# PaddleCV-SIG/MedicalSeg

Measured on AMD Instinct MI355X. Metric: 3D-voxels/sec fwd+bwd, VNet 128^3 fp32, higher is better.
Workload: dtype f32

## Files before the change

### medicalseg_amd/csrc/msk_common.h

```cpp
#pragma once
#include <hip/hip_runtime.h>
#include <hip/hip_ext.h>

#include <cstdint>
#include <cstdio>
#include <cstring>
#include <map>
#include <set>
#include <string>
#include <utility>
#include <vector>

#include "msegk.h"

struct msk_prof_entry {
  double total_ms = 0.0;
  long calls = 0;
};

struct msk_pending_event {
  hipEvent_t a, b;
  const char* tag;
};

// ... 28 lines not shown
  std::set<const void*> xform_ok;
  bool conv_fp16 = false;
  int wbf_tin_map = 1;
  int wbf_mr4 = 1;
  int wbf_variant = -1;
  int halo_tile = -1;
  int wgrad_chunk = -1;
  char prof_prefix[48] = {0};
  long wgrad_async_max_m = 0;
  float* scalar_ring = nullptr;
  int scalar_next = 0;
  long scalar_served = 0;
  float* scalar_ring_side = nullptr;
  int scalar_next_side = 0;
  long scalar_served_side = 0;
  int wbf_tpb = 0;
  void* wpack = nullptr;
  int wbf_pack_cache = 1;
  void* spack = nullptr;
  int wbf_pack_lds = 1;
  int wbf_bpf = 1;
  int wbf_ks_blocks = 2;
  int noop_after_merge = 0;
  int wgrad_c1_wpc = 2;
  int eager_tail_main = 1;
  int prof_paused = 0;
  int prof_attach = 1;
  int small_pack_cache = 1;
  int wbf_prepack = 1;
  int ks_legacy = 0;
  int wgrad_fork = 1;
  int wbf_fused_bl = 2;
  int wbf_fuse = 1;
  int conv_split = 2;
  int bwd_fuse = -1;
  int foldn_wgs = 0;
  int wgrad_wino_rounds = 0;
  int wgrad_rounds = 8;
  int poison = -1;
  hipStream_t side = nullptr;
  void* ws_side = nullptr;
  size_t ws_side_bytes = 0;
  void* ws3_side = nullptr;
  size_t ws3_side_bytes = 0;
  hipEvent_t ev_fork = nullptr, ev_join = nullptr;
  hipEvent_t ev_late = nullptr;
  bool late_valid = false;
  const float* late_ptr = nullptr;
  size_t late_count = 0;
  float* late_alpha = nullptr;
  struct { float* param = nullptr; const float* grad = nullptr; float* velocity = nullptr; size_t count = 0;
           float lr = 0, momentum = 0, weight_decay = 0, grad_scale = 0; } late_piece;
  int late_split = 1;
  bool wgrad_async = false;
  bool side_dirty = false;
  hipEvent_t fork_event = nullptr;
  int fork_attach = 1;
  bool fork_recorded = false;
  void* stage[2] = {nullptr, nullptr};
  size_t stage_bytes[2] = {0, 0};
  hipEvent_t stage_ev[2] = {nullptr, nullptr};
  int stage_next = 0;
  void* comm = nullptr;
  void* comm_grad = nullptr;
  hipStream_t comm_stream = nullptr;
  hipEvent_t ev_comm_main = nullptr, ev_comm_side = nullptr, ev_comm_done = nullptr, ev_comm_back = nullptr;
  int c1_h2 = 1;
  int dst_split = 1;
  int wgrad_reduce_rows = 1;
  int ks_stats = 1;
  int ks_lds = 1;
  int ks_nr_max = 4;
  int wgrad_lds_pad = 0;
  int kst_pair = 1;
  int tile_staging = 7;
  int wgrad_renorm = 1;
  int dy_bound_shift = 0;
  int dp_mode = 0;
  bool comm_pending = false;
  bool host_transport = false;
  std::vector<int> host_fds;
  int rank = 0, world = 1;
  int tk_join = 1;
  int affine_map = 1;
  int num_cu = 256;
};

extern thread_local std::string g_msk_global_err;

int msk_fail(msk_ctx* ctx, const char* file, int line, const char* what, const char* detail);
void* msk_workspace(msk_ctx* ctx, size_t bytes);
void* msk_workspace2(msk_ctx* ctx, size_t bytes);
void* msk_workspace3(msk_ctx* ctx, size_t bytes);
hipEvent_t msk_prof_event(msk_ctx* ctx);
void msk_prof_begin(msk_ctx* ctx, const char* tag);
void msk_prof_end(msk_ctx* ctx);
const char* msk_intern_tag(msk_ctx* ctx, const std::string& s);
int msk_join_side_impl(msk_ctx* ctx);
void msk_set_dense12(int v);
void msk_set_reduce_vpl(int v);
void msk_set_reduce_vpl_site(int v);
void msk_set_ew_caps(int ew, int red);
void msk_weights_changed_impl(msk_ctx* ctx, const void* p, size_t bytes);
void msk_weights_freed_impl(msk_ctx* ctx, const void* p, size_t bytes);
int msk_wbf_prepack_impl(msk_ctx* ctx);
int msk_wbf_prepack_range_impl(msk_ctx* ctx, const void* p, size_t bytes);
void msk_wbf_pack_cache_free(msk_ctx* ctx);
void msk_small_pack_changed(msk_ctx* ctx, const void* p, size_t bytes);
void msk_small_pack_freed(msk_ctx* ctx, const void* p, size_t bytes);
int msk_small_prepack(msk_ctx* ctx, const void* p, size_t bytes);
void msk_small_pack_free(msk_ctx* ctx);
int msk_dp_wait_impl(msk_ctx* ctx);
int msk_join_sums_merge(msk_ctx* ctx, const float* partial, int nb, int C, float* unit_sums, float* u_dbeta, float* u_dgamma,
                        float* u_dalpha, float* dalpha);

struct msk_side_scope {
  msk_ctx* ctx;
  bool active;
  explicit msk_side_scope(msk_ctx* c, bool want = true) : ctx(c), active(want && c->wgrad_async && c->side != nullptr) {
    const bool forked = ctx->fork_recorded;
    hipEvent_t fev = forked && ctx->fork_event ? ctx->fork_event : ctx->ev_fork;
    ctx->fork_recorded = false;
    ctx->fork_event = nullptr;
    if (!active) return;
    if (!forked) hipEventRecord(ctx->ev_fork, ctx->stream);
    hipStreamWaitEvent(ctx->side, fev, 0);
    std::swap(ctx->stream, ctx->side);
    std::swap(ctx->ws, ctx->ws_side);
    std::swap(ctx->ws_bytes, ctx->ws_side_bytes);
    std::swap(ctx->ws3, ctx->ws3_side);
    std::swap(ctx->ws3_bytes, ctx->ws3_side_bytes);
    std::swap(ctx->scalar_ring, ctx->scalar_ring_side);
    std::swap(ctx->scalar_next, ctx->scalar_next_side);
    std::swap(ctx->scalar_served, ctx->scalar_served_side);
    ctx->side_dirty = true;
  }
  ~msk_side_scope() {
    if (!active) return;
    std::swap(ctx->stream, ctx->side);
    std::swap(ctx->ws, ctx->ws_side);
    std::swap(ctx->ws_bytes, ctx->ws_side_bytes);
    std::swap(ctx->ws3, ctx->ws3_side);
    std::swap(ctx->ws3_bytes, ctx->ws3_side_bytes);
    std::swap(ctx->scalar_ring, ctx->scalar_ring_side);
    std::swap(ctx->scalar_next, ctx->scalar_next_side);
    std::swap(ctx->scalar_served, ctx->scalar_served_side);
  }
};

#define MSK_CHECK_HIP(ctx, expr)                                                        \
  do {                                                                                  \
    hipError_t _e = (expr);                                                             \
    if (_e != hipSuccess) return msk_fail(ctx, __FILE__, __LINE__, #expr, hipGetErrorString(_e)); \
  } while (0)

#define MSK_REQUIRE(ctx, cond, msg)                                       \
  do {                                                                    \
    if (!(cond)) return msk_fail(ctx, __FILE__, __LINE__, #cond, msg);    \
  } while (0)

static inline bool msk_prof_selected(const msk_ctx* c, const char* tag) {
  return c->prof && ((!c->prof_paused && (c->prof_prefix[0] == 0 || strncmp(tag, c->prof_prefix, strlen(c->prof_prefix)) == 0)) ||
                     strncmp(tag, "rccl_", 5) == 0);
}
struct msk_launch_scope {
  msk_ctx* ctx;
// ... 78 lines not shown
```

### medicalseg_amd/csrc/msk_conv_foldn.hip

```cpp
#include "msk_conv.h"
#include "msk_wbf.h"

typedef _Float16 fn_f16x8 __attribute__((ext_vector_type(8)));

namespace {

struct FNArgs {
  const float* src;
  int sld;
  float* dst;
  int dld;
  int N, D, H, W, CN;
  const float4* wb;
  const float* bias;
  const float* prelu;
  int accumulate;
  int tiles_h, tiles_w, segs, seg_len, nblk;
  unsigned src_bytes;
};

__device__ __forceinline__ int xcd_remap_fn(int bid, int nb) {
  const int q = nb >> 3, r = nb & 7;
  const int xcd = bid & 7, idx = bid >> 3;
  return (xcd < r ? xcd * (q + 1) : r * (q + 1) + (xcd - r) * q) + idx;
// ... 262 lines not shown
  };

  const int tap0 = wave == 0 ? 0 : NT0 - NT1 + NT1 * wave, ntap = wave == 0 ? NT0 : NT1;
  uint4 bh[NT0], bl[NT0];
  int aoff[NT0];
#pragma unroll
  for (int j = 0; j < NT0; ++j) {
    const int tp = min(tap0 + j, 24);
    bh[j] = a.wb[(tp * 2 + 0) * 64 + lane];
    bl[j] = a.wb[(tp * 2 + 1) * 64 + lane];
    aoff[j] = (tp / 5) * HW + (tp % 5);
  }
  const int abase = lk * NV + li;

  const int col_co = li / 5, col_kd = li - col_co * 5;
  const bool col_live = li < 5 * a.CN;
  const bool col_first = col_kd == 0 || !col_live;
  f32x4 acc[TH];
#pragma unroll
  for (int r = 0; r < TH; ++r) acc[r] = (f32x4){0.f, 0.f, 0.f, 0.f};

  const int steps = (d_end - d_begin) + 4;
  fetch(d_begin - 2);
#pragma unroll 1
  for (int s = 0; s < steps; ++s) {
    const int dp = d_begin - 2 + s;
    const bool live = dp >= 0 && dp < a.D;
    __syncthreads();
    if (live) {
      char* lb = reinterpret_cast<char*>(lds);
#pragma unroll
      for (int j = 0; j < NLD; ++j)
        if (st_lds[j] >= 0) {
          uint2 hv, lv;
          wbf_split2h_pair(pre[j].x * sx, pre[j].y * sx, hv.x, lv.x);
          wbf_split2h_pair(pre[j].z * sx, pre[j].w * sx, hv.y, lv.y);
          *reinterpret_cast<uint2*>(lb + st_lds[j]) = hv;
          *reinterpret_cast<uint2*>(lb + PP * 16 + st_lds[j]) = lv;
        }
    }
    __syncthreads();
    if (s + 1 < steps) fetch(dp + 1);

#pragma unroll
    for (int r = 0; r < TH; ++r)
#pragma unroll
      for (int e = 0; e < 4; ++e) {
        const float cur = acc[r][e];
        const int sh = __builtin_amdgcn_update_dpp(0, __float_as_int(cur), 0x111 , 0xF, 0xF, true);
        acc[r][e] = col_first ? 0.f : __int_as_float(sh);
      }
    if (live) {
#pragma unroll
      for (int j = 0; j < NT0; ++j) {
        if (j < ntap) {
          const uint4* ap = lds + abase + aoff[j];
#pragma unroll
          for (int r = 0; r < TH; ++r) {
            const uint4 ah = ap[r * HW], al = ap[PP + r * HW];
            acc[r] = __builtin_amdgcn_mfma_f32_16x16x32_f16(__builtin_bit_cast(fn_f16x8, al), __builtin_bit_cast(fn_f16x8, bh[j]), acc[r], 0, 0, 0);
            acc[r] = __builtin_amdgcn_mfma_f32_16x16x32_f16(__builtin_bit_cast(fn_f16x8, ah), __builtin_bit_cast(fn_f16x8, bl[j]), acc[r], 0, 0, 0);
            acc[r] = __builtin_amdgcn_mfma_f32_16x16x32_f16(__builtin_bit_cast(fn_f16x8, ah), __builtin_bit_cast(fn_f16x8, bh[j]), acc[r], 0, 0, 0);
          }
        }
      }
    }
    const int d = dp - 2;
    const bool out_plane = d >= d_begin && d < d_end;
    if (out_plane && col_live && col_kd == 4) {
#pragma unroll
      for (int r = 0; r < TH; ++r)
#pragma unroll
        for (int e = 0; e < 4; ++e) red[wave][(r * TW + 4 * lk + e) * 4 + col_co] = acc[r][e];
    }
    if (out_plane) {
      __syncthreads();
      for (int i = tid; i < TH * TW * 3; i += 256) {
        const int co = i % 3, pos = i / 3;
        const int r = pos / TW, pw = pos - r * TW;
        const int gh = h0 + r, gw = w0 + pw;
        if (co < a.CN && gh < a.H && gw < a.W) {
          const int k = pos * 4 + co;
          float v = ((red[0][k] + red[1][k]) + (red[2][k] + red[3][k])) * osc + (a.bias ? a.bias[co] : 0.f);
          float* o = a.dst + ((((long)n * a.D + d) * a.H + gh) * a.W + gw) * a.dld + co;
          if (a.accumulate) v += *o;
          if (a.prelu && v < 0.f) v *= a.prelu[co];
          *o = v;
        }
      }
    }
  }
}

}

bool msk_gconv_foldn_h2_accepts(const msk_ctx* ctx, msk_conv_desc cd, msk_tensor x, int cout) {
  if (ctx->conv_split != 2 || ctx->conv_impl != 0) return false;
  if (!(cd.kd == 5 && cd.kh == 5 && cd.kw == 5 && cd.sd == 1 && cd.sh == 1 && cd.sw == 1 && cd.pd == 2 && cd.ph == 2 && cd.pw == 2)) return false;
  if (!(x.c == 32 && cout >= 1 && 5 * cout <= 16)) return false;
  if (x.w < 12 || x.d < 4) return false;
  if (x.ld % 4 || (((uintptr_t)x.p) & 15)) return false;
  if ((size_t)x.n * x.d * x.h * x.w * x.ld * sizeof(float) >= 0xFFFFFFF0ull) return false;
  return true;
}

int msk_gconv_halo_foldn(msk_ctx* ctx, const GConv& g, const float* w_canon, int A, int B, int swap, bool* act_fused) {
  if (!(g.kd == 5 && g.kh == 5 && g.kw == 5)) return 0;
  if (!(g.sd == 1 && g.sh == 1 && g.sw == 1 && g.pd == 2 && g.ph == 2 && g.pw == 2)) return 0;
  if (!(g.SD == g.DD && g.SH == g.DH && g.SW == g.DW)) return 0;
  if (!(g.CK == 32 && g.CN >= 1 && 5 * g.CN <= 16)) return 0;
  if (g.DW < 12 || g.DD < 4) return 0;
  if (!((g.sld % 4 == 0) && (((uintptr_t)g.src) % 16 == 0))) return 0;
  constexpr int Q = 8, QG = Q / 4;
  const size_t sb = (size_t)g.N * g.SD * g.SH * g.SW * g.sld * sizeof(float);
  if (sb >= 0xFFFFFFF0ull) return 0;
  if (ctx->conv_split == 2 && ctx->conv_impl != 24) {
    unsigned short* wb2 = (unsigned short*)msk_workspace2(ctx, (size_t)25 * 2 * 64 * 8 * sizeof(unsigned short));
    if (!wb2) return -1;
    const float* x_amax = g.in_amax ? g.in_amax
                                    : msk_absmax(ctx, g.src, g.sld, g.CK, (long)g.N * g.SD * g.SH * g.SW, g.xform ? (float*)g.xform : nullptr);
    const float* w_amax = msk_absmax(ctx, w_canon, 4, 4, (125L * g.CK * g.CN + 3) / 4);
    if (!x_amax || !w_amax) return -1;
    if (g.xform) {
      if (g.in_amax)
        MSK_CHECK_HIP(ctx, hipMemcpyAsync(g.xform, g.in_amax, kWbfAmaxWays * sizeof(float), hipMemcpyDeviceToDevice, ctx->stream));
      ctx->xform_written = true;
    }
    {
      msk_launch_scope ls(ctx, "pack_weights_foldn");
      hipLaunchKernelGGL(pack_foldn_h2_weights_k, dim3(50), dim3(256), 0, ctx->stream, w_canon, A, B, swap, g.transposed ? 1 : 0, g.CN,
                         w_amax, wb2);
      MSK_LAUNCH_CHECK(ctx);
    }
    FNH2Args a{};
    a.src = g.src; a.sld = g.sld; a.dst = g.dst; a.dld = g.dld;
    a.N = g.N; a.D = g.DD; a.H = g.DH; a.W = g.DW; a.CN = g.CN;
    a.wb = (const uint4*)wb2; a.bias = g.bias; a.prelu = g.prelu; a.accumulate = g.accumulate;
    a.tiles_h = msk_cdiv(a.H, 8); a.tiles_w = msk_cdiv(a.W, 16);
    const long cols = (long)a.N * a.tiles_h * a.tiles_w;
    const long per_cu = ctx->foldn_wgs > 0 ? ctx->foldn_wgs : 3;
    int segs = (int)((per_cu * ctx->num_cu + cols - 1) / cols);
    if (segs > a.D / 8) segs = a.D / 8;
    if (segs < 1) segs = 1;
    a.seg_len = msk_cdiv(a.D, segs);
    a.segs = msk_cdiv(a.D, a.seg_len);
    const long nblk = cols * a.segs;
    if (nblk > 0x7fffffff) return 0;
    a.nblk = (int)nblk;
    a.src_bytes = (unsigned)sb;
    a.x_amax = x_amax; a.w_amax = w_amax;
    const char* tag = "conv_foldn_h2";
    if (ctx->prof && ctx->prof_shapes) {
      char buf[160];
      snprintf(buf, sizeof(buf), "conv_foldn_h2[ck=%d,cn=%d,n=%d,dhw=%dx%dx%d,acc=%d]", g.CK, g.CN, g.N, g.DD, g.DH, g.DW, g.accumulate);
      tag = msk_intern_tag(ctx, buf);
    }
    msk_launch_scope ls(ctx, tag);
    hipLaunchKernelGGL(conv_foldn_h2_k, dim3((unsigned)nblk), dim3(256), 0, ctx->stream, a);
    MSK_LAUNCH_CHECK(ctx);
    *act_fused = true;
    return 1;
  }
  float* wb = (float*)msk_workspace2(ctx, (size_t)26 * QG * 64 * 4 * sizeof(float));
  if (!wb) return -1;
  {
    msk_launch_scope ls(ctx, "pack_weights_foldn");
    hipLaunchKernelGGL(pack_foldn_weights_k, dim3(25 * QG), dim3(256), 0, ctx->stream, w_canon, A, B, swap, g.transposed ? 1 : 0,
                       g.CK, g.CN, QG, wb);
    MSK_LAUNCH_CHECK(ctx);
  }
  FNArgs a{};
  a.src = g.src; a.sld = g.sld; a.dst = g.dst; a.dld = g.dld;
  a.N = g.N; a.D = g.DD; a.H = g.DH; a.W = g.DW; a.CN = g.CN;
  a.wb = (const float4*)wb; a.bias = g.bias; a.prelu = g.prelu; a.accumulate = g.accumulate;
  a.tiles_h = msk_cdiv(a.H, 8); a.tiles_w = msk_cdiv(a.W, 16);
  const long cols = (long)a.N * a.tiles_h * a.tiles_w;
  const long per_cu = ctx->foldn_wgs > 0 ? ctx->foldn_wgs : 2;
  int segs = (int)((per_cu * ctx->num_cu + cols - 1) / cols);
  if (segs > a.D / 8) segs = a.D / 8;
  if (segs < 1) segs = 1;
  a.seg_len = msk_cdiv(a.D, segs);
  a.segs = msk_cdiv(a.D, a.seg_len);
  const long nblk = cols * a.segs;
  if (nblk > 0x7fffffff) return 0;
  a.nblk = (int)nblk;
  a.src_bytes = (unsigned)sb;
  const char* tag = "conv_foldn";
  if (ctx->prof && ctx->prof_shapes) {
    char buf[160];
    snprintf(buf, sizeof(buf), "conv_foldn[ck=%d,cn=%d,n=%d,dhw=%dx%dx%d,acc=%d]", g.CK, g.CN, g.N, g.DD, g.DH, g.DW, g.accumulate);
    tag = msk_intern_tag(ctx, buf);
  }
  msk_launch_scope ls(ctx, tag);
  hipLaunchKernelGGL((conv_foldn_k<Q>), dim3((unsigned)nblk), dim3(256), 0, ctx->stream, a);
  MSK_LAUNCH_CHECK(ctx);
  *act_fused = true;
  return 1;
}
```

### medicalseg_amd/csrc/msk_conv_tightk.hip

```cpp
#include "msk_conv.h"
#include "msk_wbf.h"

typedef _Float16 tk_f16x8 __attribute__((ext_vector_type(8)));
 __attribute__((ext_vector_type(16)));

namespace {

struct TKArgs {
  const float* src;
  int sld;
  float* dst;
  int dld;
  int N, D, H, W;
  int CN, npad;
  const float* wt;
  unsigned wt_bytes, src_bytes;
  const float* bias;
  int accumulate;
  int tiles_d, tiles_h, tiles_w, nblk;
};

__device__ __forceinline__ int xcd_remap_tk(int bid, int nb) {
  const int q = nb >> 3, r = nb & 7;
  const int xcd = bid & 7, idx = bid >> 3;
// ... 101 lines not shown
        const int l = (wave * MR + r) * 32 + row;
        const int gd = d0 + l / (TH * TW), gh = h0 + (l / TW) % TH, gw = w0 + l % TW;
        if (gd < a.D && gh < a.H && gw < a.W) {
          float* o = a.dst + ((((long)n * a.D + gd) * a.H + gh) * a.W + gw) * a.dld + co;
          float v = acc[r][j] + bv;
          if (a.accumulate) v += *o;
          *o = v;
        }
      }
    }
  }
}

template <int TD, int TH, int TW, int KS>
int launch_tk(msk_ctx* ctx, TKArgs& a, int CK, int ntn, const char* tag) {
  a.tiles_d = msk_cdiv(a.D, TD);
  a.tiles_h = msk_cdiv(a.H, TH);
  a.tiles_w = msk_cdiv(a.W, TW);
  const long nblk = (long)a.N * a.tiles_d * a.tiles_h * a.tiles_w;
  if (nblk > 0x7fffffff) return msk_fail(ctx, __FILE__, __LINE__, "conv_halo_tightk", "grid too large");
  a.nblk = (int)nblk;
  msk_launch_scope ls(ctx, tag);
  dim3 grid((unsigned)nblk, ntn);
  switch (CK) {
    case 1: hipLaunchKernelGGL((conv_halo_tightk_k<TD, TH, TW, KS, 1>), grid, dim3(256), 0, ctx->stream, a); break;
    case 2: hipLaunchKernelGGL((conv_halo_tightk_k<TD, TH, TW, KS, 2>), grid, dim3(256), 0, ctx->stream, a); break;
    case 3: hipLaunchKernelGGL((conv_halo_tightk_k<TD, TH, TW, KS, 3>), grid, dim3(256), 0, ctx->stream, a); break;
    default: hipLaunchKernelGGL((conv_halo_tightk_k<TD, TH, TW, KS, 4>), grid, dim3(256), 0, ctx->stream, a); break;
  }
  MSK_LAUNCH_CHECK(ctx);
  return 0;
}

struct TKH2Args {
  const float* src;
  int sld;
  float* dst;
  int dld;
  int N, D, H, W, CK;
  const uint4* wb;
  int accumulate;
  int tiles_h, tiles_w, segs, seg_len, nblk;
  const float* x_amax;
  const float* w_amax;
  const float* jx;
  int jxld;
  const float* jb;
  int jbld;
  float* jdb;
  int jdbld;
  const float* jcoef[6];
  float* partial;
  unsigned* maxes;
};

constexpr int kTKSteps = 16;
__global__ void __launch_bounds__(256)
pack_tkh2_weights_k(const float* __restrict__ w, int A, int B, int swap, int flip, int CK, const float* __restrict__ w_amax,
                    unsigned short* __restrict__ out) {
  const float sw = wbf_scale_of(w_amax);
  const int total = kTKSteps * 2 * 64 * 8;
  for (int idx = blockIdx.x * blockDim.x + threadIdx.x; idx < total; idx += gridDim.x * blockDim.x) {
    const int e = idx & 7, lane = (idx >> 3) & 63, nt = (idx >> 9) & 1, m = idx >> 10;
    const int n = nt * 16 + (lane & 15);
    const int u = 8 * m + 2 * (lane >> 4) + (e >> 2), c = e & 3;
    float v = 0.f;
    if (u < 125 && c < CK) {
      const int kd = u % 5, tap2 = u / 5;
      int tap = kd * 25 + tap2;
      if (flip) tap = 124 - tap;
      const int ia = swap ? n : c, ib = swap ? c : n;
      v = w[((long)ia * B + ib) * 125 + tap] * sw;
    }
    const _Float16 h = (_Float16)v;
    out[(((m * 2 + nt) * 2 + 0) * 64 + lane) * 8 + e] = __builtin_bit_cast(unsigned short, h);
    out[(((m * 2 + nt) * 2 + 1) * 64 + lane) * 8 + e] = __builtin_bit_cast(unsigned short, (_Float16)(v - (float)h));
  }
}

#ifndef TK_JOIN_PF
#define TK_JOIN_PF 1
#endif
constexpr int kTKJoinPF = TK_JOIN_PF, kTKJoinAhead = 2;
template <bool JOIN>
__global__ void __launch_bounds__(256, 3)
conv_tk_h2_k(TKH2Args a) {
  constexpr int TH = 16, TW = 16, HH = TH + 4, HW = TW + 4, NV = HH * HW;
  constexpr int RING = 8, SLOT = 2 * NV;
  constexpr int JC = RING * SLOT + 2;
  __shared__ uint2 lds[RING * SLOT + 2 + (JOIN ? 6 * 32 / 2 : 0)];
  const int tid = threadIdx.x, wave = __builtin_amdgcn_readfirstlane(tid >> 6), lane = tid & 63, li = lane & 15, lk = lane >> 4;
  int t = xcd_remap_tk(blockIdx.x, a.nblk);
  const int twi = t % a.tiles_w;
  t /= a.tiles_w;
  const int thi = t % a.tiles_h;
  t /= a.tiles_h;
  const int seg = t % a.segs;
  const int n = t / a.segs;
  const int h0 = thi * TH, w0 = twi * TW;
  const int d_begin = seg * a.seg_len;
  const int d_end = min(a.D, d_begin + a.seg_len);
  const float sx = wbf_scale_of(a.x_amax);
  const float osc = 1.f / (sx * wbf_scale_of(a.w_amax));
  constexpr int ZERO = RING * SLOT;
  if (tid == 0) lds[ZERO] = make_uint2(0u, 0u);

  long st_off[2];
  int st_v[2];
#pragma unroll
  for (int j = 0; j < 2; ++j) {
    const int v = tid + 256 * j;
    const int hh = v / HW, ww = v % HW;
    const int gh = h0 - 2 + hh, gw = w0 - 2 + ww;
    const bool inb = v < NV && gh >= 0 && gh < a.H && gw >= 0 && gw < a.W;
    st_off[j] = inb ? ((((long)n * a.D) * a.H + gh) * a.W + gw) * a.sld : -1;
    st_v[j] = v < NV ? v : -1;
  }
  const long plane = (long)a.H * a.W * a.sld;
  auto stage_load = [&](int p, float (&c)[2][4]) {
    const bool live = p >= 0 && p < a.D;
#pragma unroll
    for (int j = 0; j < 2; ++j) {
#pragma unroll
      for (int q = 0; q < 4; ++q) c[j][q] = 0.f;
      if (st_v[j] >= 0 && live && st_off[j] >= 0) {
        const float* sp = a.src + st_off[j] + (long)p * plane;
#pragma unroll
        for (int q = 0; q < 4; ++q)
          if (q < a.CK) c[j][q] = sp[q];
      }
    }
  };
  auto stage_store = [&](int p, const float (&c)[2][4]) {
    uint2* sl = lds + (p & (RING - 1)) * SLOT;
#pragma unroll
    for (int j = 0; j < 2; ++j) {
      if (st_v[j] < 0) continue;
      uint2 hv, lv;
      wbf_split2h_pair(c[j][0] * sx, c[j][1] * sx, hv.x, lv.x);
      wbf_split2h_pair(c[j][2] * sx, c[j][3] * sx, hv.y, lv.y);
      sl[st_v[j]] = hv;
      sl[NV + st_v[j]] = lv;
    }
  };

  f32x4 acc[4][2];
  const int steps = (d_end - d_begin) + 4;
  float pre[2][4];
  float js[4][2][4];
  float jm_du = 0.f, jm_xh = 0.f;
  int joff[4];
  float4 jx[8], jb[8];
  if constexpr (JOIN) {
    float* jc = reinterpret_cast<float*>(lds + JC);
    if (tid < 6 * 32) jc[tid] = a.jcoef[tid >> 5][tid & 31];
#pragma unroll
    for (int q = 0; q < 4; ++q)
#pragma unroll
      for (int nt = 0; nt < 2; ++nt)
#pragma unroll
        for (int e = 0; e < 4; ++e) js[q][nt][e] = 0.f;
#pragma unroll
    for (int r = 0; r < 4; ++r) {
      const int gh = h0 + 4 * wave + r, gw = w0 + li;
      joff[r] = (gh < a.H && gw < a.W) ? ((n * a.D) * a.H + gh) * a.W + gw : -1;
    }
  }
  const int jplane = a.H * a.W;
  auto join_load = [&](int d, int k) {
    const int r = k & 3, nt = k >> 2;
    jx[k] = make_float4(0.f, 0.f, 0.f, 0.f);
    jb[k] = make_float4(0.f, 0.f, 0.f, 0.f);
#ifndef TK_JOIN_NO_LOADS
    if (joff[r] >= 0) {
      const long v = joff[r] + d * jplane;
      jx[k] = *reinterpret_cast<const float4*>(a.jx + v * a.jxld + 16 * nt + 4 * lk);
      jb[k] = *reinterpret_cast<const float4*>(a.jb + v * a.jbld + 16 * nt + 4 * lk);
    }
#endif
  };
  auto join_chunk = [&](int d, int k) {
    const int r = k & 3, nt = k >> 2;
    if (joff[r] < 0) return;
    const float4* jc4 = reinterpret_cast<const float4*>(lds + JC);
    const float4 c0 = jc4[0 * 8 + 4 * nt + lk], c1 = jc4[1 * 8 + 4 * nt + lk], c2 = jc4[2 * 8 + 4 * nt + lk];
    const float4 c3 = jc4[3 * 8 + 4 * nt + lk], c4 = jc4[4 * 8 + 4 * nt + lk], c5 = jc4[5 * 8 + 4 * nt + lk];
    const float sc[4] = {c0.x, c0.y, c0.z, c0.w}, sf[4] = {c1.x, c1.y, c1.z, c1.w}, ai[4] = {c2.x, c2.y, c2.z, c2.w};
    const float al[4] = {c3.x, c3.y, c3.z, c3.w}, mu[4] = {c4.x, c4.y, c4.z, c4.w}, is[4] = {c5.x, c5.y, c5.z, c5.w};
    const float xv[4] = {jx[k].x, jx[k].y, jx[k].z, jx[k].w}, rv[4] = {jb[k].x, jb[k].y, jb[k].z, jb[k].w};
    float du[4];
#pragma unroll
    for (int j = 0; j < 4; ++j) {
      const float dv = acc[r][nt][j] * osc;
      float t = fmaf(xv[j], sc[j], sf[j]);
      const float tin = t;
      if (!(t > 0.f)) t *= ai[j];
      const float u = t + rv[j];
      t = tin;
      float g = dv;
      if (!(u > 0.f)) {
        g = al[j] * dv;
        js[3][nt][j] = fmaf(dv, u, js[3][nt][j]);
      }
      du[j] = g;
      float gu = g;
      if (!(t > 0.f)) {
        gu = g * ai[j];
        js[2][nt][j] = fmaf(g, fmaf(xv[j], sc[j], sf[j]), js[2][nt][j]);
      }
      const float xh = (xv[j] - mu[j]) * is[j];
      js[0][nt][j] += gu;
      js[1][nt][j] = fmaf(gu, xh, js[1][nt][j]);
      jm_du = fmaxf(jm_du, fabsf(gu));
      jm_xh = fmaxf(jm_xh, fabsf(xh));
    }
    const long v = joff[r] + d * jplane;
    *reinterpret_cast<float4*>(a.dst + v * a.dld + 16 * nt + 4 * lk) = make_float4(du[0], du[1], du[2], du[3]);
    if (a.jdb) *reinterpret_cast<float4*>(a.jdb + v * a.jdbld + 16 * nt + 4 * lk) = make_float4(du[0], du[1], du[2], du[3]);
  };
#pragma unroll 1
  for (int s = 0; s < 5; ++s) {
    stage_load(d_begin - 2 + s, pre);
    stage_store(d_begin - 2 + s, pre);
  }
  __syncthreads();
#pragma unroll 1
  for (int s = 4; s < steps; ++s) {
    const int d = d_begin + s - 4;
    stage_load(d + 3, pre);
    if constexpr (JOIN) {
#pragma unroll
      for (int k = 0; k < kTKJoinPF; ++k) join_load(d, k);
    }
#pragma unroll
    for (int r = 0; r < 4; ++r)
#pragma unroll
      for (int nt = 0; nt < 2; ++nt) acc[r][nt] = (f32x4){0.f, 0.f, 0.f, 0.f};
    const int dring = (d - 2) & (RING - 1);
#pragma unroll 2
    for (int m = 0; m < kTKSteps; ++m) {
      uint4 wf[2][2];
#pragma unroll
      for (int nt = 0; nt < 2; ++nt)
#pragma unroll
        for (int pc = 0; pc < 2; ++pc) wf[nt][pc] = a.wb[((m * 2 + nt) * 2 + pc) * 64 + lane];
      int b0, b1, st0, st1, lo0, lo1;
      {
        const int u0 = 8 * m + 2 * lk, u1 = u0 + 1;
        const int t0 = u0 / 5, t1 = u1 / 5;
        const int k0 = u0 - 5 * t0, k1 = u1 - 5 * t1;
        const int v0 = (4 * wave + t0 / 5) * HW + li + t0 % 5, v1 = (4 * wave + t1 / 5) * HW + li + t1 % 5;
        const bool z0 = u0 >= 125, z1 = u1 >= 125;
        b0 = z0 ? ZERO : ((dring + k0) & (RING - 1)) * SLOT + v0;
        b1 = z1 ? ZERO : ((dring + k1) & (RING - 1)) * SLOT + v1;
        st0 = z0 ? 0 : HW; st1 = z1 ? 0 : HW; lo0 = z0 ? 0 : NV; lo1 = z1 ? 0 : NV;
      }
      uint4 xh[4], xl[4];
#pragma unroll
      for (int r = 0; r < 4; ++r) {
        const uint2 h0v = lds[b0 + r * st0], h1v = lds[b1 + r * st1];
        const uint2 l0v = lds[b0 + lo0 + r * st0], l1v = lds[b1 + lo1 + r * st1];
        xh[r] = make_uint4(h0v.x, h0v.y, h1v.x, h1v.y);
        xl[r] = make_uint4(l0v.x, l0v.y, l1v.x, l1v.y);
      }
#pragma unroll
      for (int r = 0; r < 4; ++r)
#pragma unroll
        for (int nt = 0; nt < 2; ++nt)
          acc[r][nt] = __builtin_amdgcn_mfma_f32_16x16x32_f16(__builtin_bit_cast(tk_f16x8, wf[nt][1]), __builtin_bit_cast(tk_f16x8, xh[r]), acc[r][nt], 0, 0, 0);
#pragma unroll
      for (int r = 0; r < 4; ++r)
#pragma unroll
        for (int nt = 0; nt < 2; ++nt)
          acc[r][nt] = __builtin_amdgcn_mfma_f32_16x16x32_f16(__builtin_bit_cast(tk_f16x8, wf[nt][0]), __builtin_bit_cast(tk_f16x8, xl[r]), acc[r][nt], 0, 0, 0);
#pragma unroll
      for (int r = 0; r < 4; ++r)
#pragma unroll
        for (int nt = 0; nt < 2; ++nt)
          acc[r][nt] = __builtin_amdgcn_mfma_f32_16x16x32_f16(__builtin_bit_cast(tk_f16x8, wf[nt][0]), __builtin_bit_cast(tk_f16x8, xh[r]), acc[r][nt], 0, 0, 0);
    }
    if constexpr (JOIN) {
#pragma unroll
      for (int k = kTKJoinPF; k < kTKJoinPF + kTKJoinAhead && k < 8; ++k) join_load(d, k);
#pragma unroll
      for (int k = 0; k < 8; ++k) {
        if (k >= kTKJoinPF && k + kTKJoinAhead < 8) join_load(d, k + kTKJoinAhead);
        join_chunk(d, k);
        __builtin_amdgcn_sched_barrier(0);
      }
    } else if (d < d_end) {
#pragma unroll
      for (int r = 0; r < 4; ++r) {
        const int gh = h0 + 4 * wave + r, gw = w0 + li;
        if (gh < a.H && gw < a.W) {
          float* o = a.dst + ((((long)n * a.D + d) * a.H + gh) * a.W + gw) * a.dld + 4 * lk;
#pragma unroll
          for (int nt = 0; nt < 2; ++nt) {
            float4 v = make_float4(acc[r][nt][0] * osc, acc[r][nt][1] * osc, acc[r][nt][2] * osc, acc[r][nt][3] * osc);
            float4* op = reinterpret_cast<float4*>(o + 16 * nt);
            if (a.accumulate) {
              const float4 e = *op;
              v.x += e.x; v.y += e.y; v.z += e.z; v.w += e.w;
            }
            *op = v;
          }
        }
      }
    }
    stage_store(d + 3, pre);
    __syncthreads();
  }
  if constexpr (JOIN) {
    float* red = reinterpret_cast<float*>(lds);
#pragma unroll
    for (int q = 0; q < 4; ++q)
#pragma unroll
      for (int nt = 0; nt < 2; ++nt)
#pragma unroll
        for (int e = 0; e < 4; ++e) {
          float v = js[q][nt][e];
#pragma unroll
          for (int o = 8; o > 0; o >>= 1) v += __shfl_xor(v, o);
          if (li == 0) red[(wave * 4 + q) * 32 + 16 * nt + 4 * lk + e] = v;
        }
    __syncthreads();
    if (tid < 4 * 32) {
      const float v = ((red[tid] + red[128 + tid]) + red[256 + tid]) + red[384 + tid];
      a.partial[(long)blockIdx.x * 128 + tid] = v;
    }
    block_atomic_max(a.maxes, jm_du);
    block_atomic_max(a.maxes + kWbfAmaxWays, jm_xh);
  }
}

}

bool msk_gconv_tk_h2_accepts(const msk_ctx* ctx, const GConv& g, const TKJoin* join) {
  if (ctx->conv_split != 2 || ctx->conv_impl == 25) return false;
  if (!(g.kd == 5 && g.kh == 5 && g.kw == 5 && g.sd == 1 && g.sh == 1 && g.sw == 1 && g.pd == 2 && g.ph == 2 && g.pw == 2)) return false;
  if (!(g.SD == g.DD && g.SH == g.DH && g.SW == g.DW)) return false;
  if (g.CK < 1 || g.CK > 4 || g.CN != 32 || g.bias || g.prelu) return false;
  if (g.DW < 12 || g.DH < 8 || g.DD < 4) return false;
  if (g.dld % 4 || (((uintptr_t)g.dst) & 15)) return false;
  if (join) {
    if (!ctx->tk_join || g.accumulate) return false;
    if (join->xld % 4 || join->bld % 4 || (((uintptr_t)join->x) & 15) || (((uintptr_t)join->b) & 15)) return false;
    if (join->db && (join->dbld % 4 || (((uintptr_t)join->db) & 15))) return false;
    if (!(join->scale && join->shift && join->alpha_in && join->alpha && join->mean && join->invstd && join->maxes)) return false;
  }
  return true;
}

int msk_gconv_tk_h2(msk_ctx* ctx, const GConv& g, const float* w_canon, int A, int B, int swap, TKJoin* join) {
  if (!msk_gconv_tk_h2_accepts(ctx, g, join)) return 0;
  unsigned short* wb = (unsigned short*)msk_workspace2(ctx, (size_t)kTKSteps * 2 * 2 * 64 * 8 * sizeof(unsigned short));
  if (!wb) return -1;
  const float* x_amax = g.in_amax ? g.in_amax : msk_absmax(ctx, g.src, g.sld, g.CK, (long)g.N * g.SD * g.SH * g.SW);
  const float* w_amax = msk_absmax(ctx, w_canon, 4, 4, (125L * g.CK * g.CN + 3) / 4);
  if (!x_amax || !w_amax) return -1;
  {
    msk_launch_scope ls(ctx, "pack_weights_tightk");
    hipLaunchKernelGGL(pack_tkh2_weights_k, dim3(100), dim3(256), 0, ctx->stream, w_canon, A, B, swap, g.transposed ? 1 : 0, g.CK, w_amax, wb);
    MSK_LAUNCH_CHECK(ctx);
  }
  TKH2Args a{};
  a.src = g.src; a.sld = g.sld; a.dst = g.dst; a.dld = g.dld;
  a.N = g.N; a.D = g.DD; a.H = g.DH; a.W = g.DW; a.CK = g.CK;
  a.wb = (const uint4*)wb; a.accumulate = g.accumulate;
  a.tiles_h = msk_cdiv(a.H, 16); a.tiles_w = msk_cdiv(a.W, 16);
  const long cols = (long)a.N * a.tiles_h * a.tiles_w;
  const long per_cu = ctx->foldn_wgs > 0 ? ctx->foldn_wgs : 3;
  int segs = (int)((per_cu * ctx->num_cu + cols - 1) / cols);
  if (segs > a.D / 8) segs = a.D / 8;
  if (segs < 1) segs = 1;
  a.seg_len = msk_cdiv(a.D, segs);
  a.segs = msk_cdiv(a.D, a.seg_len);
  const long nblk = cols * a.segs;
  if (nblk > 0x7fffffff) return 0;
  a.nblk = (int)nblk;
  a.x_amax = x_amax; a.w_amax = w_amax;
  if (join) {
    float* partial = (float*)msk_workspace(ctx, (size_t)nblk * 4 * 32 * sizeof(float));
    if (!partial) return -1;
    a.jx = join->x; a.jxld = join->xld; a.jb = join->b; a.jbld = join->bld; a.jdb = join->db; a.jdbld = join->dbld;
    a.jcoef[0] = join->scale; a.jcoef[1] = join->shift; a.jcoef[2] = join->alpha_in;
    a.jcoef[3] = join->alpha; a.jcoef[4] = join->mean; a.jcoef[5] = join->invstd;
    a.partial = partial; a.maxes = (unsigned*)join->maxes;
    join->partial = partial; join->nb = a.nblk;
  }
  const char* tag = join ? "conv_tk_h2_join" : "conv_tk_h2";
  if (ctx->prof && ctx->prof_shapes) {
    char buf[160];
    snprintf(buf, sizeof(buf), "%s[ck=%d,cn=%d,n=%d,dhw=%dx%dx%d,acc=%d]", tag, g.CK, g.CN, g.N, g.DD, g.DH, g.DW, g.accumulate);
    tag = msk_intern_tag(ctx, buf);
  }
  msk_launch_scope ls(ctx, tag);
  if (join) hipLaunchKernelGGL(conv_tk_h2_k<true>, dim3((unsigned)nblk), dim3(256), 0, ctx->stream, a);
  else hipLaunchKernelGGL(conv_tk_h2_k<false>, dim3((unsigned)nblk), dim3(256), 0, ctx->stream, a);
  MSK_LAUNCH_CHECK(ctx);
  return 1;
}

int msk_gconv_halo_tightk(msk_ctx* ctx, const GConv& g, const float* w_canon, int A, int B, int swap) {
  const int ks = g.kd;
  if (!(g.kd == g.kh && g.kh == g.kw && ks == 5)) return 0;
  if (!(g.sd == 1 && g.sh == 1 && g.sw == 1 && g.pd == 2 && g.ph == 2 && g.pw == 2)) return 0;
  if (!(g.SD == g.DD && g.SH == g.DH && g.SW == g.DW)) return 0;
  if (g.CK < 2 || g.CK > 4 || g.CN < 8) return 0;
  const int taps = ks * ks * ks, HT = (taps + 1) / 2;
  const int npad = ((g.CN + 31) / 32) * 32;
  float* wt = (float*)msk_workspace2(ctx, (size_t)HT * g.CK * 2 * npad * sizeof(float));
  if (!wt) return -1;
  {
    msk_launch_scope ls(ctx, "pack_weights_tightk");
    hipLaunchKernelGGL(pack_tightk_weights_k, dim3(64), dim3(256), 0, ctx->stream, w_canon, A, B, ks, swap,
                       g.transposed ? 1 : 0, g.CK, g.CN, npad, wt);
    MSK_LAUNCH_CHECK(ctx);
  }
  TKArgs a{};
  a.src = g.src; a.sld = g.sld; a.dst = g.dst; a.dld = g.dld;
  a.N = g.N; a.D = g.DD; a.H = g.DH; a.W = g.DW;
  a.CN = g.CN; a.npad = npad; a.wt = wt; a.bias = g.bias; a.accumulate = g.accumulate;
  a.wt_bytes = (unsigned)((size_t)HT * g.CK * 2 * npad * sizeof(float));
  {
    const size_t sb = (size_t)g.N * g.SD * g.SH * g.SW * g.sld * sizeof(float);
    if (sb >= 0xFFFFFFF0ull) return 0;
    a.src_bytes = (unsigned)sb;
  }
  const char* tag = "conv_halo_tightk";
  if (ctx->prof && ctx->prof_shapes) {
    char buf[160];
    snprintf(buf, sizeof(buf), "conv_halo_tightk[ck=%d,cn=%d,n=%d,dhw=%dx%dx%d,acc=%d]", g.CK, g.CN, g.N, g.DD, g.DH, g.DW,
             g.accumulate);
    tag = msk_intern_tag(ctx, buf);
  }
  int rc;
  if (g.DW >= 32 && g.DW % 32 < 1) rc = launch_tk<2, 4, 32, 5>(ctx, a, g.CK, npad / 32, tag);
  else if (g.DW >= 16 && g.DW % 16 < 1) rc = launch_tk<2, 8, 16, 5>(ctx, a, g.CK, npad / 32, tag);
  else rc = launch_tk<4, 8, 8, 5>(ctx, a, g.CK, npad / 32, tag);
  return rc == 0 ? 1 : rc;
}
```

### medicalseg_amd/csrc/msk_ctx.hip

```cpp
#include <cstdlib>

#include "msk_common.h"

thread_local std::string g_msk_global_err;

int msk_fail(msk_ctx* ctx, const char* file, int line, const char* what, const char* detail) {
  char buf[1024];
  const char* base = strrchr(file, '/');
  snprintf(buf, sizeof(buf), "%s:%d: %s: %s", base ? base + 1 : file, line, what, detail ? detail : "");
  if (ctx) ctx->err = buf;
  g_msk_global_err = buf;
  return -1;
}

static void* grow(msk_ctx* ctx, void** p, size_t* cur, size_t bytes) {
  if (bytes <= *cur) return *p;
  if (*p) {
    hipStreamSynchronize(ctx->stream);
    hipFree(*p);
    *p = nullptr;
    *cur = 0;
  }
  size_t want = bytes + (bytes >> 2);
  if (hipMalloc(p, want) != hipSuccess) {
// ... 495 lines not shown
    ctx->ks_lds = value;
    return 0;
  }
  if (strcmp(key, "dense12") == 0) {
    msk_set_dense12(value);
    return 0;
  }
  if (strcmp(key, "reduce_vpl") == 0) {
    msk_set_reduce_vpl(value);
    return 0;
  }
  if (strcmp(key, "reduce_vpl_site") == 0) {
    msk_set_reduce_vpl_site(value);
    return 0;
  }
  if (strcmp(key, "reduce_cap") == 0) {
    msk_set_ew_caps(0, value);
    return 0;
  }
  if (strcmp(key, "dy_bound_shift") == 0) {
    ctx->dy_bound_shift = value;
    return 0;
  }
  if (strcmp(key, "late_split") == 0) {
    ctx->late_split = value != 0;
    return 0;
  }
  if (strcmp(key, "c1_h2") == 0) {
    ctx->c1_h2 = value < 0 ? 0 : (value > 2 ? 2 : value);
    return 0;
  }
  if (strcmp(key, "ks_nr_max") == 0) {
    ctx->ks_nr_max = value >= 4 ? 4 : (value >= 2 ? 2 : 1);
    return 0;
  }
  if (strcmp(key, "wgrad_lds_pad") == 0) {
    ctx->wgrad_lds_pad = value > 0 ? value : 0;
    return 0;
  }
  if (strcmp(key, "kst_pair") == 0) {
    ctx->kst_pair = value != 0;
    return 0;
  }
  if (strcmp(key, "tile_staging") == 0) {
    ctx->tile_staging = value;
    return 0;
  }
  if (strcmp(key, "wgrad_renorm") == 0) {
    ctx->wgrad_renorm = value != 0;
    return 0;
  }
  if (strcmp(key, "ks_legacy") == 0) {
    ctx->ks_legacy = value;
    return 0;
  }
  if (strcmp(key, "wgrad_fork") == 0) {
    ctx->wgrad_fork = value;
    return 0;
  }
  if (strcmp(key, "wbf_fuse") == 0) {
    ctx->wbf_fuse = value;
    return 0;
  }
  if (strcmp(key, "wbf_fused_bl") == 0) {
    ctx->wbf_fused_bl = value;
    return 0;
  }
  if (strcmp(key, "wbf_tpb") == 0) {
    ctx->wbf_tpb = value > 0 ? value : 0;
    return 0;
  }
  if (strcmp(key, "conv_split") == 0) {
    ctx->conv_split = value == 2 ? 2 : 3;
    return 0;
  }
  if (strcmp(key, "bwd_fuse") == 0) {
    ctx->bwd_fuse = value < 0 ? -1 : (value > 2 ? 2 : value);
    return 0;
  }
  if (strcmp(key, "tk_join") == 0) {
    ctx->tk_join = value != 0;
    return 0;
  }
  if (strcmp(key, "affine_map") == 0) {
    ctx->affine_map = value != 0;
    return 0;
  }
  if (strcmp(key, "foldn_wgs") == 0) {
    ctx->foldn_wgs = value > 0 ? value : 0;
    return 0;
  }
  if (strcmp(key, "wgrad_wino_rounds") == 0) {
    ctx->wgrad_wino_rounds = value > 0 ? value : 0;
    return 0;
  }
  if (strcmp(key, "wgrad_rounds") == 0) {
    ctx->wgrad_rounds = value > 0 ? value : 8;
    return 0;
  }
  if (strcmp(key, "wgrad_chunk") == 0) {
    ctx->wgrad_chunk = value;
    return 0;
  }
  if (strcmp(key, "wgrad_async") == 0) {
    if (msk_join_side_impl(ctx) != 0) return -1;
    ctx->wgrad_async = value != 0;
    return 0;
  }
  if (strcmp(key, "prof_shapes") == 0) {
    ctx->prof_shapes = value != 0;
    return 0;
  }
  if (strcmp(key, "poison_scratch") == 0) {
    ctx->poison = value;
    if (value >= 0) {
      hipStreamSynchronize(ctx->stream);
      if (ctx->ws) hipMemsetAsync(ctx->ws, value, ctx->ws_bytes, ctx->stream);
      if (ctx->ws2) hipMemsetAsync(ctx->ws2, value, ctx->ws2_bytes, ctx->stream);
    }
    return 0;
  }
  return msk_fail(ctx, __FILE__, __LINE__, "msk_set_option", "unknown key");
}

}
```

Measured before the change: 251.3 million.

## Add row-split foldn kernel and table-driven LDS addressing in tightk conv

Adds a new foldn h2 kernel variant. Its kw=4 tap column is computed from a separate LDS weight copy with extra row accumulators and reduced through a fifth reduction slot, which rebalances MFMA work across waves. Also adds a tightk h2 variant that precomputes per-step LDS unit offsets into a double-buffered table and reads the operands with inline ds_read_b64 using immediate offsets. Ring slots are padded to spread LDS banks. Both paths are on by default, at the cost of more LDS, extra registers, and hand-written asm with a full lgkmcnt wait.

```diff
diff --git a/medicalseg_amd/csrc/msk_common.h b/medicalseg_amd/csrc/msk_common.h
--- a/medicalseg_amd/csrc/msk_common.h
+++ b/medicalseg_amd/csrc/msk_common.h
@@ -134,6 +134,8 @@
   std::vector<int> host_fds;
   int rank = 0, world = 1;
   int tk_join = 1;
+  int foldn_rows = 1;
+  int tk_tables = 1;
   int affine_map = 1;
   int num_cu = 256;
 };
diff --git a/medicalseg_amd/csrc/msk_conv_foldn.hip b/medicalseg_amd/csrc/msk_conv_foldn.hip
--- a/medicalseg_amd/csrc/msk_conv_foldn.hip
+++ b/medicalseg_amd/csrc/msk_conv_foldn.hip
@@ -368,6 +368,178 @@
         if (co < a.CN && gh < a.H && gw < a.W) {
           const int k = pos * 4 + co;
           float v = ((red[0][k] + red[1][k]) + (red[2][k] + red[3][k])) * osc + (a.bias ? a.bias[co] : 0.f);
+          float* o = a.dst + ((((long)n * a.D + d) * a.H + gh) * a.W + gw) * a.dld + co;
+          if (a.accumulate) v += *o;
+          if (a.prelu && v < 0.f) v *= a.prelu[co];
+          *o = v;
+        }
+      }
+    }
+  }
+}
+
+
+__global__ void __launch_bounds__(256, 3)
+conv_foldn_h2_rows_k(FNH2Args a) {
+  constexpr int TH = 8, TW = 16, HH = TH + 4, HW = TW + 4, NV = HH * HW;
+  constexpr int NW = 4, NT = 64 * NW;
+  constexpr int NLD = (NV * 8 + NT - 1) / NT;
+  constexpr unsigned kOOB = 0xFFFFFFF0u;
+  constexpr int PP = 4 * NV;
+  __shared__ uint4 lds[2 * PP];
+  __shared__ float red[NW + 1][TH * TW * 4];
+  __shared__ uint4 wl[5 * 2 * 64];
+
+  const int tid = threadIdx.x, wave = __builtin_amdgcn_readfirstlane(tid >> 6), lane = tid & 63, li = lane & 15, lk = lane >> 4;
+  int t = xcd_remap_fn(blockIdx.x, a.nblk);
+  const int twi = t % a.tiles_w;
+  t /= a.tiles_w;
+  const int thi = t % a.tiles_h;
+  t /= a.tiles_h;
+  const int seg = t % a.segs;
+  const int n = t / a.segs;
+  const int h0 = thi * TH, w0 = twi * TW;
+  const int d_begin = seg * a.seg_len;
+  const int d_end = min(a.D, d_begin + a.seg_len);
+  const float sx = wbf_scale_of(a.x_amax);
+  const float osc = 1.f / (sx * wbf_scale_of(a.w_amax));
+
+  const __amdgpu_buffer_rsrc_t sres = __builtin_amdgcn_make_buffer_rsrc((void*)a.src, 0, a.src_bytes, 0x00020000);
+  unsigned st_off[NLD];
+  const int st_v0 = 8 * wave + (li >> 1), st_q = 2 * lk + (li & 1);
+  const int st_lds0 = (lk * NV + st_v0) * 16 + (li & 1) * 8;
+  const bool st_last = st_v0 + 8 * NW * (NLD - 1) < NV;
+#pragma unroll
+  for (int j = 0; j < NLD; ++j) {
+    const int v = st_v0 + 8 * NW * j;
+    const int hh = v / HW, ww = v % HW;
+    const int gh = h0 - 2 + hh, gw = w0 - 2 + ww;
+    const bool inb = v < NV && gh >= 0 && gh < a.H && gw >= 0 && gw < a.W;
+    st_off[j] = inb ? (unsigned)(((((long)n * a.D * a.H + gh) * a.W + gw) * a.sld + 4 * st_q) * 4) : kOOB;
+  }
+  const long plane_bytes = (long)a.H * a.W * a.sld * 4;
+  float4 pre[NLD];
+  auto fetch = [&](int dp) {
+    const bool live = dp >= 0 && dp < a.D;
+    const unsigned soff = live ? (unsigned)(dp * plane_bytes) : 0u;
+#pragma unroll
+    for (int j = 0; j < NLD; ++j)
+      pre[j] = live ? __builtin_bit_cast(float4, __builtin_amdgcn_raw_buffer_load_b128(sres, (int)st_off[j], (int)soff, 0))
+                    : make_float4(0.f, 0.f, 0.f, 0.f);
+  };
+
+  uint4 bh[5], bl[5];
+#pragma unroll
+  for (int kh = 0; kh < 5; ++kh) {
+    bh[kh] = a.wb[((kh * 5 + wave) * 2 + 0) * 64 + lane];
+    bl[kh] = a.wb[((kh * 5 + wave) * 2 + 1) * 64 + lane];
+  }
+  const uint4* ap = lds + lk * NV + li + wave;
+  const uint4* ap4 = lds + lk * NV + li + 4 + 2 * wave * HW;
+  for (int i = tid; i < 5 * 2 * 64; i += NT) wl[i] = a.wb[(((i >> 7) * 5 + 4) * 2 + ((i >> 6) & 1)) * 64 + (i & 63)];
+  f32x4 accx[2];
+  accx[0] = accx[1] = (f32x4){0.f, 0.f, 0.f, 0.f};
+
+  const int col_co = li / 5, col_kd = li - col_co * 5;
+  const bool col_live = li < 5 * a.CN;
+  const bool col_first = col_kd == 0 || !col_live;
+  f32x4 acc[TH];
+#pragma unroll
+  for (int r = 0; r < TH; ++r) acc[r] = (f32x4){0.f, 0.f, 0.f, 0.f};
+
+  const int steps = (d_end - d_begin) + 4;
+  fetch(d_begin - 2);
+#pragma unroll 1
+  for (int s = 0; s < steps; ++s) {
+    const int dp = d_begin - 2 + s;
+    const bool live = dp >= 0 && dp < a.D;
+    __syncthreads();
+    if (live) {
+      char* lb = reinterpret_cast<char*>(lds) + st_lds0;
+#pragma unroll
+      for (int j = 0; j < NLD; ++j) {
+        if (j == NLD - 1 && !st_last) continue;
+        uint2 hv, lv;
+        wbf_split2h_pair(pre[j].x * sx, pre[j].y * sx, hv.x, lv.x);
+        wbf_split2h_pair(pre[j].z * sx, pre[j].w * sx, hv.y, lv.y);
+        *reinterpret_cast<uint2*>(lb + j * (8 * NW * 16)) = hv;
+        *reinterpret_cast<uint2*>(lb + PP * 16 + j * (8 * NW * 16)) = lv;
+      }
+    }
+    __syncthreads();
+    if (s + 1 < steps) fetch(dp + 1);
+
+#pragma unroll
+    for (int r = 0; r < TH; ++r)
+#pragma unroll
+      for (int e = 0; e < 4; ++e) {
+        const float cur = acc[r][e];
+        const int sh = __builtin_amdgcn_update_dpp(0, __float_as_int(cur), 0x111 , 0xF, 0xF, true);
+        acc[r][e] = col_first ? 0.f : __int_as_float(sh);
+      }
+#pragma unroll
+    for (int r = 0; r < 2; ++r)
+#pragma unroll
+      for (int e = 0; e < 4; ++e) {
+        const float cur = accx[r][e];
+        const int sh = __builtin_amdgcn_update_dpp(0, __float_as_int(cur), 0x111 , 0xF, 0xF, true);
+        accx[r][e] = col_first ? 0.f : __int_as_float(sh);
+      }
+    if (live) {
+#pragma unroll
+      for (int j = 0; j < 6; ++j) {
+        const fn_f16x8 ah = __builtin_bit_cast(fn_f16x8, ap4[j * HW]), al = __builtin_bit_cast(fn_f16x8, ap4[PP + j * HW]);
+#pragma unroll
+        for (int r = 0; r < 2; ++r)
+          if (j - r >= 0 && j - r < 5)
+            accx[r] = __builtin_amdgcn_mfma_f32_16x16x32_f16(al, __builtin_bit_cast(fn_f16x8, wl[((j - r) * 2 + 0) * 64 + lane]), accx[r], 0, 0, 0);
+#pragma unroll
+        for (int r = 0; r < 2; ++r)
+          if (j - r >= 0 && j - r < 5)
+            accx[r] = __builtin_amdgcn_mfma_f32_16x16x32_f16(ah, __builtin_bit_cast(fn_f16x8, wl[((j - r) * 2 + 1) * 64 + lane]), accx[r], 0, 0, 0);
+#pragma unroll
+        for (int r = 0; r < 2; ++r)
+          if (j - r >= 0 && j - r < 5)
+            accx[r] = __builtin_amdgcn_mfma_f32_16x16x32_f16(ah, __builtin_bit_cast(fn_f16x8, wl[((j - r) * 2 + 0) * 64 + lane]), accx[r], 0, 0, 0);
+      }
+#pragma unroll
+      for (int j = 0; j < HH; ++j) {
+        const fn_f16x8 ah = __builtin_bit_cast(fn_f16x8, ap[j * HW]), al = __builtin_bit_cast(fn_f16x8, ap[PP + j * HW]);
+#pragma unroll
+        for (int kh = 0; kh < 5; ++kh)
+          if (j - kh >= 0 && j - kh < TH)
+            acc[j - kh] = __builtin_amdgcn_mfma_f32_16x16x32_f16(al, __builtin_bit_cast(fn_f16x8, bh[kh]), acc[j - kh], 0, 0, 0);
+#pragma unroll
+        for (int kh = 0; kh < 5; ++kh)
+          if (j - kh >= 0 && j - kh < TH)
+            acc[j - kh] = __builtin_amdgcn_mfma_f32_16x16x32_f16(ah, __builtin_bit_cast(fn_f16x8, bl[kh]), acc[j - kh], 0, 0, 0);
+#pragma unroll
+        for (int kh = 0; kh < 5; ++kh)
+          if (j - kh >= 0 && j - kh < TH)
+            acc[j - kh] = __builtin_amdgcn_mfma_f32_16x16x32_f16(ah, __builtin_bit_cast(fn_f16x8, bh[kh]), acc[j - kh], 0, 0, 0);
+      }
+    }
+    const int d = dp - 2;
+    const bool out_plane = d >= d_begin && d < d_end;
+    if (out_plane && col_live && col_kd == 4) {
+#pragma unroll
+      for (int r = 0; r < TH; ++r)
+#pragma unroll
+        for (int e = 0; e < 4; ++e) red[wave][(r * TW + 4 * lk + e) * 4 + col_co] = acc[r][e];
+#pragma unroll
+      for (int r = 0; r < 2; ++r)
+#pragma unroll
+        for (int e = 0; e < 4; ++e) red[NW][((2 * wave + r) * TW + 4 * lk + e) * 4 + col_co] = accx[r][e];
+    }
+    if (out_plane) {
+      __syncthreads();
+      for (int i = tid; i < TH * TW * 3; i += NT) {
+        const int co = i % 3, pos = i / 3;
+        const int r = pos / TW, pw = pos - r * TW;
+        const int gh = h0 + r, gw = w0 + pw;
+        if (co < a.CN && gh < a.H && gw < a.W) {
+          const int k = pos * 4 + co;
+          float v = (((red[0][k] + red[1][k]) + (red[2][k] + red[3][k])) + red[4][k]) * osc + (a.bias ? a.bias[co] : 0.f);
           float* o = a.dst + ((((long)n * a.D + d) * a.H + gh) * a.W + gw) * a.dld + co;
           if (a.accumulate) v += *o;
           if (a.prelu && v < 0.f) v *= a.prelu[co];
@@ -438,11 +610,15 @@
     const char* tag = "conv_foldn_h2";
     if (ctx->prof && ctx->prof_shapes) {
       char buf[160];
-      snprintf(buf, sizeof(buf), "conv_foldn_h2[ck=%d,cn=%d,n=%d,dhw=%dx%dx%d,acc=%d]", g.CK, g.CN, g.N, g.DD, g.DH, g.DW, g.accumulate);
+      snprintf(buf, sizeof(buf), "conv_foldn_h2[ck=%d,cn=%d,n=%d,dhw=%dx%dx%d,acc=%d,rows=%d]", g.CK, g.CN, g.N, g.DD, g.DH, g.DW, g.accumulate,
+               ctx->foldn_rows);
       tag = msk_intern_tag(ctx, buf);
     }
     msk_launch_scope ls(ctx, tag);
-    hipLaunchKernelGGL(conv_foldn_h2_k, dim3((unsigned)nblk), dim3(256), 0, ctx->stream, a);
+    const dim3 grid((unsigned)nblk);
+    if (ctx->foldn_rows) hipLaunchKernelGGL(conv_foldn_h2_rows_k, grid, dim3(256), 0, ctx->stream, a);
+    else
+      hipLaunchKernelGGL(conv_foldn_h2_k, dim3((unsigned)nblk), dim3(256), 0, ctx->stream, a);
     MSK_LAUNCH_CHECK(ctx);
     *act_fused = true;
     return 1;
diff --git a/medicalseg_amd/csrc/msk_conv_tightk.hip b/medicalseg_amd/csrc/msk_conv_tightk.hip
--- a/medicalseg_amd/csrc/msk_conv_tightk.hip
+++ b/medicalseg_amd/csrc/msk_conv_tightk.hip
@@ -207,13 +207,38 @@
 #define TK_JOIN_PF 1
 #endif
 constexpr int kTKJoinPF = TK_JOIN_PF, kTKJoinAhead = 2;
-template <bool JOIN>
+typedef unsigned long long tk_u64;
+__device__ __forceinline__ void tk_read_step(unsigned a0, unsigned a1, uint4 (&xh)[4], uint4 (&xl)[4]) {
+  tk_u64 h0[4], h1[4], l0[4], l1[4];
+  asm volatile(
+      "ds_read_b64 %0, %16\n\tds_read_b64 %1, %17\n\t"
+      "ds_read_b64 %2, %16 offset:160\n\tds_read_b64 %3, %17 offset:160\n\t"
+      "ds_read_b64 %4, %16 offset:320\n\tds_read_b64 %5, %17 offset:320\n\t"
+      "ds_read_b64 %6, %16 offset:480\n\tds_read_b64 %7, %17 offset:480\n\t"
+      "ds_read_b64 %8, %16 offset:3200\n\tds_read_b64 %9, %17 offset:3200\n\t"
+      "ds_read_b64 %10, %16 offset:3360\n\tds_read_b64 %11, %17 offset:3360\n\t"
+      "ds_read_b64 %12, %16 offset:3520\n\tds_read_b64 %13, %17 offset:3520\n\t"
+      "ds_read_b64 %14, %16 offset:3680\n\tds_read_b64 %15, %17 offset:3680\n\t"
+      "s_waitcnt lgkmcnt(0)"
+      : "=&v"(h0[0]), "=&v"(h1[0]), "=&v"(h0[1]), "=&v"(h1[1]), "=&v"(h0[2]), "=&v"(h1[2]), "=&v"(h0[3]), "=&v"(h1[3]),
+        "=&v"(l0[0]), "=&v"(l1[0]), "=&v"(l0[1]), "=&v"(l1[1]), "=&v"(l0[2]), "=&v"(l1[2]), "=&v"(l0[3]), "=&v"(l1[3])
+      : "v"(a0), "v"(a1)
+      : "memory");
+#pragma unroll
+  for (int r = 0; r < 4; ++r) {
+    xh[r] = make_uint4((unsigned)h0[r], (unsigned)(h0[r] >> 32), (unsigned)h1[r], (unsigned)(h1[r] >> 32));
+    xl[r] = make_uint4((unsigned)l0[r], (unsigned)(l0[r] >> 32), (unsigned)l1[r], (unsigned)(l1[r] >> 32));
+  }
+}
+template <bool JOIN, bool TAB>
 __global__ void __launch_bounds__(256, 3)
 conv_tk_h2_k(TKH2Args a) {
   constexpr int TH = 16, TW = 16, HH = TH + 4, HW = TW + 4, NV = HH * HW;
-  constexpr int RING = 8, SLOT = 2 * NV;
-  constexpr int JC = RING * SLOT + 2;
-  __shared__ uint2 lds[RING * SLOT + 2 + (JOIN ? 6 * 32 / 2 : 0)];
+  constexpr int RING = 8, SLOT = 2 * NV + (TAB ? 8 : 0);
+  static_assert(!TAB || SLOT % 32 == 8, "bank spreading of the ring slots");
+  constexpr int TB = RING * SLOT;
+  constexpr int JC = RING * SLOT + (TAB ? 64 : 2);
+  __shared__ uint2 lds[JC + (JOIN ? 6 * 32 / 2 : 0)];
   const int tid = threadIdx.x, wave = __builtin_amdgcn_readfirstlane(tid >> 6), lane = tid & 63, li = lane & 15, lk = lane >> 4;
   int t = xcd_remap_tk(blockIdx.x, a.nblk);
   const int twi = t % a.tiles_w;
@@ -228,7 +253,22 @@
   const float sx = wbf_scale_of(a.x_amax);
   const float osc = 1.f / (sx * wbf_scale_of(a.w_amax));
   constexpr int ZERO = RING * SLOT;
-  if (tid == 0) lds[ZERO] = make_uint2(0u, 0u);
+  if (!TAB && tid == 0) lds[ZERO] = make_uint2(0u, 0u);
+  auto fill_tab = [&](int dring, int buf) {
+    if (tid < 64) {
+      unsigned e = 0;
+#pragma unroll
+      for (int j = 0; j < 2; ++j) {
+        const int u = min(2 * tid + j, 124);
+        const int tp = u / 5, kd = u - 5 * tp;
+        e |= (unsigned)((((dring + kd) & (RING - 1)) * SLOT + (tp / 5) * HW + tp % 5) * 8) << (16 * j);
+      }
+      reinterpret_cast<unsigned*>(lds + TB)[buf * 64 + tid] = e;
+    }
+  };
+  static_assert((RING * SLOT + 2 * NV) * 8 < 65536, "a unit's byte offset fits 16 bits");
+  static_assert(HW * 8 == 160 && NV * 8 == 3200, "the immediate offsets of tk_read_step");
+  const unsigned lbase = (unsigned)(unsigned long)(__attribute__((address_space(3))) void*)lds + (4 * wave * HW + li) * 8;
 
   long st_off[2];
   int st_v[2];
@@ -348,6 +388,7 @@
     stage_load(d_begin - 2 + s, pre);
     stage_store(d_begin - 2 + s, pre);
   }
+  if constexpr (TAB) fill_tab((d_begin - 2) & (RING - 1), 0);
   __syncthreads();
 #pragma unroll 1
   for (int s = 4; s < steps; ++s) {
@@ -362,6 +403,9 @@
 #pragma unroll
       for (int nt = 0; nt < 2; ++nt) acc[r][nt] = (f32x4){0.f, 0.f, 0.f, 0.f};
     const int dring = (d - 2) & (RING - 1);
+    const unsigned* tb = reinterpret_cast<const unsigned*>(lds + TB) + (s & 1) * 64 + lk;
+    unsigned en = 0;
+    if constexpr (TAB) en = tb[0];
 #pragma unroll 2
     for (int m = 0; m < kTKSteps; ++m) {
       uint4 wf[2][2];
@@ -369,8 +413,11 @@
       for (int nt = 0; nt < 2; ++nt)
 #pragma unroll
         for (int pc = 0; pc < 2; ++pc) wf[nt][pc] = a.wb[((m * 2 + nt) * 2 + pc) * 64 + lane];
-      int b0, b1, st0, st1, lo0, lo1;
-      {
+      int b0 = 0, b1 = 0, st0 = 0, st1 = 0, lo0 = 0, lo1 = 0;
+      const unsigned e01 = en;
+      if constexpr (TAB) {
+        en = tb[((m + 1) & (kTKSteps - 1)) * 4];
+      } else {
         const int u0 = 8 * m + 2 * lk, u1 = u0 + 1;
         const int t0 = u0 / 5, t1 = u1 / 5;
         const int k0 = u0 - 5 * t0, k1 = u1 - 5 * t1;
@@ -381,8 +428,9 @@
         st0 = z0 ? 0 : HW; st1 = z1 ? 0 : HW; lo0 = z0 ? 0 : NV; lo1 = z1 ? 0 : NV;
       }
       uint4 xh[4], xl[4];
-#pragma unroll
-      for (int r = 0; r < 4; ++r) {
+      if constexpr (TAB) tk_read_step(lbase + (e01 & 0xFFFFu), lbase + (e01 >> 16), xh, xl);
+#pragma unroll
+      for (int r = 0; r < 4 && !TAB; ++r) {
         const uint2 h0v = lds[b0 + r * st0], h1v = lds[b1 + r * st1];
         const uint2 l0v = lds[b0 + lo0 + r * st0], l1v = lds[b1 + lo1 + r * st1];
         xh[r] = make_uint4(h0v.x, h0v.y, h1v.x, h1v.y);
@@ -433,6 +481,7 @@
       }
     }
     stage_store(d + 3, pre);
+    if constexpr (TAB) fill_tab((d - 1) & (RING - 1), (s + 1) & 1);
     __syncthreads();
   }
   if constexpr (JOIN) {
@@ -516,12 +565,16 @@
   const char* tag = join ? "conv_tk_h2_join" : "conv_tk_h2";
   if (ctx->prof && ctx->prof_shapes) {
     char buf[160];
-    snprintf(buf, sizeof(buf), "%s[ck=%d,cn=%d,n=%d,dhw=%dx%dx%d,acc=%d]", tag, g.CK, g.CN, g.N, g.DD, g.DH, g.DW, g.accumulate);
+    snprintf(buf, sizeof(buf), "%s[ck=%d,cn=%d,n=%d,dhw=%dx%dx%d,acc=%d,tab=%d]", tag, g.CK, g.CN, g.N, g.DD, g.DH, g.DW, g.accumulate,
+             ctx->tk_tables);
     tag = msk_intern_tag(ctx, buf);
   }
   msk_launch_scope ls(ctx, tag);
-  if (join) hipLaunchKernelGGL(conv_tk_h2_k<true>, dim3((unsigned)nblk), dim3(256), 0, ctx->stream, a);
-  else hipLaunchKernelGGL(conv_tk_h2_k<false>, dim3((unsigned)nblk), dim3(256), 0, ctx->stream, a);
+  const dim3 grid((unsigned)nblk), block(256);
+  if (join && ctx->tk_tables) hipLaunchKernelGGL((conv_tk_h2_k<true, true>), grid, block, 0, ctx->stream, a);
+  else if (join) hipLaunchKernelGGL((conv_tk_h2_k<true, false>), grid, block, 0, ctx->stream, a);
+  else if (ctx->tk_tables) hipLaunchKernelGGL((conv_tk_h2_k<false, true>), grid, block, 0, ctx->stream, a);
+  else hipLaunchKernelGGL((conv_tk_h2_k<false, false>), grid, block, 0, ctx->stream, a);
   MSK_LAUNCH_CHECK(ctx);
   return 1;
 }
diff --git a/medicalseg_amd/csrc/msk_ctx.hip b/medicalseg_amd/csrc/msk_ctx.hip
--- a/medicalseg_amd/csrc/msk_ctx.hip
+++ b/medicalseg_amd/csrc/msk_ctx.hip
@@ -601,6 +601,14 @@
     ctx->tk_join = value != 0;
     return 0;
   }
+  if (strcmp(key, "foldn_rows") == 0) {
+    ctx->foldn_rows = value != 0;
+    return 0;
+  }
+  if (strcmp(key, "tk_tables") == 0) {
+    ctx->tk_tables = value != 0;
+    return 0;
+  }
   if (strcmp(key, "affine_map") == 0) {
     ctx->affine_map = value != 0;
     return 0;
```

After: 249.0 million. No clear change (-0.9%).
